# theodorblackbird/lina-speech

Hardware: AMD Instinct MI355X
Metric: codec tokens/sec (whole node), 169M d1024xl12 batched greedy decode (higher is better)
Workload: dtype bf16

## Files before the change

### lina-speech_amd/csrc/gla_decode_window.hip

```cpp
#include <lina_dev.h>
#include "lina_common.h"
#include "skinny_frag.h"

#ifndef LINA_K1W_HIST_NT
#define LINA_K1W_HIST_NT 0
#endif

#ifndef LINA_K1W_STATE_PLAIN
#define LINA_K1W_STATE_PLAIN 0
#endif
#ifndef LINA_K1W_NO_TAIL_LOADS
#define LINA_K1W_NO_TAIL_LOADS 0
#endif
#if LINA_K1W_STATE_PLAIN
#define LINA_K1W_STATE_LOAD(p) (*reinterpret_cast<const float4*>(p))
#else
#define LINA_K1W_STATE_LOAD(p) ld_nt4(p)
#endif

namespace lina {

constexpr int kWinMax = 16;

__device__ __forceinline__ float ld_hist(const float* p) {
#if LINA_K1W_HIST_NT
    return ld_nt1(p);
#else
    return *p;
#endif
}
__device__ __forceinline__ void st_hist(float* p, float v) {
#if LINA_K1W_HIST_NT
    st_nt1(p, v);
#else
    *p = v;
#endif
}

template <typename TS> struct state_piece { static constexpr int n = 4; };
template <> struct state_piece<bf16_t> { static constexpr int n = 8; };
__device__ __forceinline__ void ld_state(const float* p, float (&x)[4]) {
    const float4 t = LINA_K1W_STATE_LOAD(p);
    x[0] = t.x; x[1] = t.y; x[2] = t.z; x[3] = t.w;
}
__device__ __forceinline__ void ld_state(const bf16_t* p, float (&x)[8]) {
    const uint4 u = ld_nt16(p);
    const float4 lo = cvt4(make_uint2(u.x, u.y)), hi = cvt4(make_uint2(u.z, u.w));
    x[0] = lo.x; x[1] = lo.y; x[2] = lo.z; x[3] = lo.w; x[4] = hi.x; x[5] = hi.y; x[6] = hi.z; x[7] = hi.w;
}
__device__ __forceinline__ void st_state(float* p, const float (&x)[4]) { st_nt4(p, make_float4(x[0], x[1], x[2], x[3])); }
__device__ __forceinline__ void st_state(bf16_t* p, const float (&x)[8]) {
    st_nt16(p, make_uint4(pack_bf16x2(x[0], x[1]), pack_bf16x2(x[2], x[3]), pack_bf16x2(x[4], x[5]), pack_bf16x2(x[6], x[7])));
}

template <int DV, int NRB, int CS, typename TIO, typename TG, typename TS = float>
__global__ __launch_bounds__(256 * NRB) void gla_decode_window_kernel(
    const TIO* __restrict__ q, const TIO* __restrict__ k, const TIO* __restrict__ v, const TG* __restrict__ gk, TS* S,
    float* hist_k, float* hist_c, float* hist_v, const int64_t* step, const int64_t* origin, int window, int flush_n,
    int H, int64_t q_sb, int64_t q_sh, int64_t k_sb, int64_t k_sh, int64_t v_sb, int64_t v_sh, int64_t g_sb,
    int64_t g_sh, float scale, const TIO* __restrict__ gate, int64_t gate_sb, int64_t gate_sh,
    const TIO* __restrict__ nw, float eps, TIO* __restrict__ og, int og_packed, float* o_x, int* counters) {
    constexpr int DVT = DV * CS;
    constexpr int RB = 64;
    constexpr int DK = RB * NRB;
    constexpr int EPL = state_piece<TS>::n;
    constexpr int CG = DV / EPL;
    constexpr int RPI = 256 / CG;
    constexpr int NP = RB / RPI;
    __shared__ float s_q[DK], s_e[DK], s_a[kWinMax][NRB];
    __shared__ float s_w[kWinMax][DK];
    __shared__ __attribute__((aligned(16))) float s_v[kWinMax][DV];
    __shared__ __attribute__((aligned(16))) float s_red[NRB * RPI * DV];

    const int tid = threadIdx.x;
    const int rb = tid >> 8, t256 = tid & 255;
    const int cg = t256 % CG, rg = t256 / CG;
    const int bh = blockIdx.x, b = bh / H, h = bh % H;
    const int r0 = rb * RB;
    const int64_t BH = gridDim.x;
    const int col0 = CS > 1 ? (int)blockIdx.y * DV : 0;
    TS* tile = S + ((int64_t)bh * DK + r0) * DVT + col0 + EPL * cg;

    const bool flush_only = flush_n >= 0;
    const int j = flush_only ? flush_n - 1 : ((int)(step[0] - origin[0]) & (window - 1));
    const bool write_back = flush_only || j == window - 1;
    if (flush_only && flush_n == 0) return;

    const int n_hist = flush_only ? j + 1 : j;
    constexpr int NV = 192 * NRB;
    const bool row_wave = t256 < RB;
    float h1[kWinMax], h2[kWinMax];
    float gj = 0.f, kj = 0.f, qj = 0.f, vj = 0.f;
    const int row = r0 + (t256 & (RB - 1));
    const int64_t hoff = (int64_t)bh * DK + row;
    const int vc = rb * 192 + t256 - RB;
    if (row_wave) {
#pragma unroll
        for (int s = 0; s < kWinMax; ++s) {
            h1[s] = s < n_hist ? ld_hist(&hist_c[(int64_t)s * BH * DK + hoff]) : 0.0f;
            h2[s] = s < n_hist ? ld_hist(&hist_k[(int64_t)s * BH * DK + hoff]) : 0.0f;
        }
        if (!flush_only) {
            gj = ld(gk + b * g_sb + h * g_sh + row);
            kj = ld(k + b * k_sb + h * k_sh + row);
            qj = ld(q + b * q_sb + h * q_sh + row) * scale;
        }
    } else if (vc < DV) {
#pragma unroll
        for (int s = 0; s < kWinMax; ++s) h1[s] = s < n_hist ? ld_hist(&hist_v[((int64_t)s * BH + bh) * DVT + col0 + vc]) : 0.0f;
        if (!flush_only) vj = ld(v + b * v_sb + h * v_sh + col0 + vc);
    }

    float St[NP][EPL];
#pragma unroll
    for (int i = 0; i < NP; ++i) ld_state(tile + (int64_t)(rg + RPI * i) * DVT, St[i]);

    if (row_wave) {
        float cj;
        if (flush_only) {
            cj = h1[kWinMax - 1];
#pragma unroll
            for (int s = 0; s < kWinMax - 1; ++s) cj = (s == j) ? h1[s] : cj;
        } else {
            float cprev = 0.0f;
#pragma unroll
            for (int s = 0; s < kWinMax; ++s) cprev = (s == j - 1) ? h1[s] : cprev;
            cj = cprev + gj;
            if (CS == 1 || blockIdx.y == 0) {
                st_hist(&hist_c[(int64_t)j * BH * DK + hoff], cj);
                st_hist(&hist_k[(int64_t)j * BH * DK + hoff], kj);
            }
        }
        s_q[row] = qj;
        s_e[row] = __expf(cj);
#pragma unroll
        for (int s = 0; s < kWinMax; ++s) {
            if (s <= j) {
                const float ws = (!flush_only && s == j) ? kj : __expf(cj - h1[s]) * h2[s];
                s_w[s][row] = ws;
                float a = qj * ws;
                a += shfl_xor(a, 1); a += shfl_xor(a, 2); a += shfl_xor(a, 4);
                a += shfl_xor(a, 8); a += shfl_xor(a, 16); a += shfl_xor(a, 32);
                if (t256 == 0) s_a[s][rb] = a;
            }
        }
    } else {
        if (vc < DV) {
#pragma unroll
            for (int s = 0; s < kWinMax; ++s)
                if (s <= j) s_v[s][vc] = (!flush_only && s == j) ? vj : h1[s];
            if (!flush_only) st_hist(&hist_v[((int64_t)j * BH + bh) * DVT + col0 + vc], vj);
        }
        for (int c = vc + NV; c < DV; c += NV) {
            for (int s = 0; s <= j; ++s) {
                float vs;
                if (!flush_only && s == j) {
                    vs = ld(v + b * v_sb + h * v_sh + col0 + c);
                    hist_v[((int64_t)j * BH + bh) * DVT + col0 + c] = vs;
                } else {
                    vs = hist_v[((int64_t)s * BH + bh) * DVT + col0 + c];
                }
                s_v[s][c] = vs;
            }
        }
    }
    __syncthreads();

    float acc[EPL];
#pragma unroll
    for (int e = 0; e < EPL; ++e) acc[e] = 0.f;
    if (write_back) {
#pragma unroll
        for (int i = 0; i < NP; ++i) {
            const float d = s_e[r0 + rg + RPI * i];
#pragma unroll
            for (int e = 0; e < EPL; ++e) St[i][e] *= d;
        }
        for (int s = 0; s <= j; ++s) {
            float vv[EPL];
#pragma unroll
            for (int e4 = 0; e4 < EPL; e4 += 4) {
                const float4 t = *reinterpret_cast<const float4*>(&s_v[s][EPL * cg + e4]);
                vv[e4] = t.x; vv[e4 + 1] = t.y; vv[e4 + 2] = t.z; vv[e4 + 3] = t.w;
            }
#pragma unroll
            for (int i = 0; i < NP; ++i) {
                const float ws = s_w[s][r0 + rg + RPI * i];
#pragma unroll
                for (int e = 0; e < EPL; ++e) St[i][e] = fmaf(ws, vv[e], St[i][e]);
            }
        }
#pragma unroll
        for (int i = 0; i < NP; ++i) st_state(tile + (int64_t)(rg + RPI * i) * DVT, St[i]);
        if (flush_only) return;
#pragma unroll
        for (int i = 0; i < NP; ++i) {
            const float qq = s_q[r0 + rg + RPI * i];
#pragma unroll
            for (int e = 0; e < EPL; ++e) acc[e] = fmaf(qq, St[i][e], acc[e]);
        }
    } else {
#pragma unroll
        for (int i = 0; i < NP; ++i) {
            const int rr = r0 + rg + RPI * i;
            const float qe = s_q[rr] * s_e[rr];
#pragma unroll
            for (int e = 0; e < EPL; ++e) acc[e] = fmaf(qe, St[i][e], acc[e]);
        }
    }
#pragma unroll
    for (int e4 = 0; e4 < EPL; e4 += 4)
        *reinterpret_cast<float4*>(&s_red[(rb * RPI + rg) * DV + EPL * cg + e4]) = make_float4(acc[e4], acc[e4 + 1], acc[e4 + 2], acc[e4 + 3]);
    __syncthreads();
    if (tid < 64) {
        constexpr int CG4 = DV / 4;
        float4 r = make_float4(0.f, 0.f, 0.f, 0.f);
        if (tid < CG4) {
            r = *reinterpret_cast<const float4*>(&s_red[4 * tid]);
#pragma unroll
            for (int jj = 1; jj < NRB * RPI; ++jj) {
                const float4 t = *reinterpret_cast<const float4*>(&s_red[jj * DV + 4 * tid]);
                r.x += t.x; r.y += t.y; r.z += t.z; r.w += t.w;
            }
            if (!write_back)
                for (int s = 0; s <= j; ++s) {
                    float a = s_a[s][0];
#pragma unroll
                    for (int g2 = 1; g2 < NRB; ++g2) a += s_a[s][g2];
                    const float4 vv = *reinterpret_cast<const float4*>(&s_v[s][4 * tid]);
                    r.x = fmaf(a, vv.x, r.x); r.y = fmaf(a, vv.y, r.y); r.z = fmaf(a, vv.z, r.z); r.w = fmaf(a, vv.w, r.w);
                }
        }
        float ss = r.x * r.x + r.y * r.y + r.z * r.z + r.w * r.w;
        ss += shfl_xor(ss, 1); ss += shfl_xor(ss, 2); ss += shfl_xor(ss, 4);
        ss += shfl_xor(ss, 8); ss += shfl_xor(ss, 16); ss += shfl_xor(ss, 32);
        auto finish = [&](float4 x, int c0, float rs) {
            if (tid < CG4) {
                x.x *= rs; x.y *= rs; x.z *= rs; x.w *= rs;
#if LINA_K1W_NO_TAIL_LOADS
                const float4 ww = make_float4(1.f, 1.f, 1.f, 1.f), gg = make_float4(eps, scale, eps, scale);
#else
                const float4 ww = ld4(nw + c0 + 4 * tid);
                const float4 gg = ld4(gate + b * gate_sb + h * gate_sh + c0 + 4 * tid);
#endif
                x.x *= ww.x; x.y *= ww.y; x.z *= ww.z; x.w *= ww.w;
                x.x *= gg.x * sigmoidf(gg.x); x.y *= gg.y * sigmoidf(gg.y);
                x.z *= gg.z * sigmoidf(gg.z); x.w *= gg.w * sigmoidf(gg.w);
                if (og_packed) st4(og + packed_off<TIO>(b, h * DVT + c0 + 4 * tid, H * DVT), x);
                else st4(og + (int64_t)bh * DVT + c0 + 4 * tid, x);
            }
        };
        if constexpr (CS == 1) {
            finish(r, 0, rsqrtf(ss / (float)DV + eps));
        } else {
            float* ox = o_x + (int64_t)bh * DVT;
            if (tid < CG4) { st_agent8(ox + col0 + 4 * tid, r.x, r.y); st_agent8(ox + col0 + 4 * tid + 2, r.z, r.w); }
            drain_stores();
            int t = 0;
            if (tid == 0) t = ticket_agent(&counters[bh]);
            t = shfl_i(t, 0);
            if (t == CS - 1) {
                if (tid == 0) counters[bh] = 0;
                float4 oth[CS];
                float tot = ss;
#pragma unroll
                for (int c = 0; c < CS; ++c) {
                    oth[c] = r;
                    if (c != (int)blockIdx.y) {
                        float4 x = make_float4(0.f, 0.f, 0.f, 0.f);
                        if (tid < CG4) {
                            const float2 lo = ld_agent8(ox + c * DV + 4 * tid), hi = ld_agent8(ox + c * DV + 4 * tid + 2);
                            x = make_float4(lo.x, lo.y, hi.x, hi.y);
                        }
                        float s2 = x.x * x.x + x.y * x.y + x.z * x.z + x.w * x.w;
                        s2 += shfl_xor(s2, 1); s2 += shfl_xor(s2, 2); s2 += shfl_xor(s2, 4);
                        s2 += shfl_xor(s2, 8); s2 += shfl_xor(s2, 16); s2 += shfl_xor(s2, 32);
                        tot += s2;
                        oth[c] = x;
                    }
                }
                const float rs = rsqrtf(tot / (float)DVT + eps);
#pragma unroll
                for (int c = 0; c < CS; ++c) finish(oth[c], c * DV, rs);
            }
        }
    }
}

constexpr int kWinPersist = 8;
template <typename T> __device__ __forceinline__ T* at_byte(T* base, int byte_off) {
    opaque(byte_off);
    return (T*)((const char*)base + (unsigned)byte_off);
}

template <int DV, int NRB, int CS, typename TIO, typename TG, typename TS = float>
__global__ __launch_bounds__(256 * NRB) void gla_decode_window_persist_kernel(
    const TIO* __restrict__ q, const TIO* __restrict__ k, const TIO* __restrict__ v, const TG* __restrict__ gk, TS* S,
    float* hist_k, float* hist_c, float* hist_v, const int64_t* step, const int64_t* origin, int window, int n_heads,
    int H, int64_t q_sb, int64_t q_sh, int64_t k_sb, int64_t k_sh, int64_t v_sb, int64_t v_sh, int64_t g_sb,
    int64_t g_sh, float scale, const TIO* __restrict__ gate, int64_t gate_sb, int64_t gate_sh,
    const TIO* __restrict__ nw, float eps, TIO* __restrict__ og, int og_packed) {
    static_assert(CS == 1, "the persistent form serves heads of one column block");
    constexpr int RB = 64;
    constexpr int DK = RB * NRB;
    constexpr int EPL = state_piece<TS>::n;
    constexpr int CG = DV / EPL;
    constexpr int RPI = 256 / CG;
    constexpr int NP = RB / RPI;
    constexpr int RD = NP >= 2 ? NP / 2 : 1;
    constexpr int PG = RD < 4 ? RD : 4;
    static_assert(NP % RD == 0 && RD % PG == 0, "a head is a whole number of passes over the ring");
    constexpr int CG4 = DV / 4;
    constexpr int NH = kWinPersist - 1;
    struct __attribute__((aligned(16))) head_lds {
        __attribute__((aligned(16))) float v[kWinPersist][DV];
        __attribute__((aligned(16))) float red[NRB * RPI * DV];
        float w[kWinPersist][DK];
        float q[DK], e[DK], a[kWinPersist][NRB];
        typename raw4<TIO>::type gate[CG4];
    };
    __shared__ head_lds s_buf[2];
    __shared__ typename raw4<TIO>::type s_nw[CG4];

    const int tid = threadIdx.x;
    const int rb = tid >> 8, t256 = tid & 255;
    const int cg = t256 % CG, rg = t256 / CG;
    const int r0 = rb * RB;
    const int64_t BH = n_heads;
    const int n_wg = (int)gridDim.x;
    int bh = blockIdx.x;
    if (bh >= n_heads) return;

    const int j = (int)(step[0] - origin[0]) & (window - 1);
    const bool write_back = j == window - 1;
    const int n_hist = j;
    const int s_last = n_hist > 0 ? n_hist - 1 : 0;
    constexpr int NV = 192 * NRB;
    const bool row_wave = wave_uniform(t256 < RB ? 1 : 0) != 0;
    const int row = r0 + (t256 & (RB - 1));
    const int vc = rb * 192 + t256 - RB;
    const int vcc = vc < 0 ? 0 : (vc < DV ? vc : DV - 1);
    const int toff = ((r0 + rg) * DV + EPL * cg) * (int)sizeof(TS);
    const int hoffl = (row_wave ? row : vcc) * 4;
    const int rowio = row * (int)sizeof(TIO), rowg = row * (int)sizeof(TG), vcio = vcc * (int)sizeof(TIO);
    const int t4io = (tid & (CG4 - 1)) * 4 * (int)sizeof(TIO);
    int pstep_ = RPI * DV;
    opaque(pstep_);
    const int pstep = wave_uniform(pstep_);
    const float* hA = row_wave ? hist_c : hist_v;
    const float* hB = row_wave ? hist_k : hist_v;
    const int64_t hw = row_wave ? DK : DV;

    float h1[NH], h2[NH];
    decltype(ld_raw(gk)) gj_r;
    decltype(ld_raw(q)) kj_r, qj_r, vj_r;
    typename raw4<TIO>::type gate_r;
    if (tid < CG4) s_nw[tid] = ld4_raw(nw + 4 * tid);
    auto small_loads = [&](int hd) __attribute__((always_inline)) {
        const int b = hd / H, h = hd % H;
#pragma unroll
        for (int s = 0; s < NH; ++s) {
            const int sc = s < n_hist ? s : s_last;
            const int64_t o = ((int64_t)sc * BH + hd) * hw;
            h1[s] = ld_hist(at_byte(hA + o, hoffl));
            h2[s] = ld_hist(at_byte(hB + o, hoffl));
        }
        gj_r = ld_raw(at_byte(gk + (b * g_sb + h * g_sh), rowg));
        kj_r = ld_raw(at_byte(k + (b * k_sb + h * k_sh), rowio));
        qj_r = ld_raw(at_byte(q + (b * q_sb + h * q_sh), rowio));
        vj_r = ld_raw(at_byte(v + (b * v_sb + h * v_sh), vcio));
        gate_r = ld4_raw(at_byte(gate + (b * gate_sb + h * gate_sh), t4io));
    };

    float St[RD][EPL];
    small_loads(bh);
    {
        const TS* tile = S + (int64_t)bh * DK * DV;
#pragma unroll
        for (int i = 0; i < RD; ++i) ld_state(at_byte(tile + i * pstep, toff), St[i]);
    }

    auto head = [&](const bool WB, const bool NEXT, const int p, const int nx) __attribute__((always_inline)) {
        const int b = bh / H, h = bh % H;
        const int64_t hoff = (int64_t)bh * DK;
        head_lds& L = s_buf[p];
        if (tid < CG4) L.gate[tid] = gate_r;
        if (row_wave) {
            const float gj = cvt1(gj_r), kj = cvt1(kj_r), qj = cvt1(qj_r) * scale;
            float cprev = 0.0f;
#pragma unroll
            for (int s = 0; s < NH; ++s) cprev = (s == j - 1) ? h1[s] : cprev;
            const float cj = cprev + gj;
            st_hist(at_byte(hist_c + ((int64_t)j * BH * DK + hoff), row * 4), cj);
            st_hist(at_byte(hist_k + ((int64_t)j * BH * DK + hoff), row * 4), kj);
            L.q[row] = qj;
            L.e[row] = __expf(cj);
#pragma unroll
            for (int s = 0; s < kWinPersist; ++s) {
                if (s <= j) {
                    const float ws = (s == j) ? kj : __expf(cj - h1[s < NH ? s : 0]) * h2[s < NH ? s : 0];
                    L.w[s][row] = ws;
                    float a = qj * ws;
                    a += shfl_xor(a, 1); a += shfl_xor(a, 2); a += shfl_xor(a, 4);
                    a += shfl_xor(a, 8); a += shfl_xor(a, 16); a += shfl_xor(a, 32);
                    if (t256 == 0) L.a[s][rb] = a;
                }
            }
        } else {
            if (vc < DV) {
                const float vj = cvt1(vj_r);
#pragma unroll
                for (int s = 0; s < kWinPersist; ++s)
                    if (s <= j) L.v[s][vc] = (s == j) ? vj : h1[s < NH ? s : 0];
                st_hist(at_byte(hist_v + ((int64_t)j * BH + bh) * DV, vc * 4), vj);
            }
            for (int c = vc + NV; c < DV; c += NV) {
                for (int s = 0; s <= j; ++s) {
                    float vs;
                    if (s == j) {
                        vs = ld(v + b * v_sb + h * v_sh + c);
                        hist_v[((int64_t)j * BH + bh) * DV + c] = vs;
                    } else {
                        vs = hist_v[((int64_t)s * BH + bh) * DV + c];
                    }
                    L.v[s][c] = vs;
                }
            }
        }
        __syncthreads();

        small_loads(NEXT ? nx : bh);
        TS* tile = S + (int64_t)bh * DK * DV;
        const TS* tile_nx = NEXT ? S + (int64_t)nx * DK * DV : tile;
        const int pstep_nx = NEXT ? pstep : 0;

        float acc[EPL];
#pragma unroll
        for (int e = 0; e < EPL; ++e) acc[e] = 0.f;
#pragma unroll
        for (int g0 = 0; g0 < NP; g0 += PG) {
            const int sl = g0 % RD;
            if (WB) {
#pragma unroll
                for (int u = 0; u < PG; ++u) {
                    const float d = L.e[r0 + rg + RPI * (g0 + u)];
#pragma unroll
                    for (int e = 0; e < EPL; ++e) St[sl + u][e] *= d;
                }
                for (int s = 0; s <= j; ++s) {
                    float vv[EPL];
#pragma unroll
                    for (int e4 = 0; e4 < EPL; e4 += 4) {
                        const float4 t = *reinterpret_cast<const float4*>(&L.v[s][EPL * cg + e4]);
                        vv[e4] = t.x; vv[e4 + 1] = t.y; vv[e4 + 2] = t.z; vv[e4 + 3] = t.w;
                    }
#pragma unroll
                    for (int u = 0; u < PG; ++u) {
                        const float ws = L.w[s][r0 + rg + RPI * (g0 + u)];
#pragma unroll
                        for (int e = 0; e < EPL; ++e) St[sl + u][e] = fmaf(ws, vv[e], St[sl + u][e]);
                    }
                }
#pragma unroll
                for (int u = 0; u < PG; ++u) st_state(at_byte(tile + (g0 + u) * pstep, toff), St[sl + u]);
#pragma unroll
                for (int u = 0; u < PG; ++u) {
                    const float qq = L.q[r0 + rg + RPI * (g0 + u)];
#pragma unroll
                    for (int e = 0; e < EPL; ++e) acc[e] = fmaf(qq, St[sl + u][e], acc[e]);
                }
            } else {
#pragma unroll
                for (int u = 0; u < PG; ++u) {
                    const int rr = r0 + rg + RPI * (g0 + u);
                    const float qe = L.q[rr] * L.e[rr];
#pragma unroll
                    for (int e = 0; e < EPL; ++e) acc[e] = fmaf(qe, St[sl + u][e], acc[e]);
                }
            }
            if (g0 + RD < NP) {
#pragma unroll
                for (int u = 0; u < PG; ++u) ld_state(at_byte(tile + (g0 + RD + u) * pstep, toff), St[sl + u]);
            } else {
#pragma unroll
                for (int u = 0; u < PG; ++u) ld_state(at_byte(tile_nx + (g0 + RD - NP + u) * pstep_nx, toff), St[sl + u]);
            }
        }
#pragma unroll
        for (int e4 = 0; e4 < EPL; e4 += 4)
            *reinterpret_cast<float4*>(&L.red[(rb * RPI + rg) * DV + EPL * cg + e4]) = make_float4(acc[e4], acc[e4 + 1], acc[e4 + 2], acc[e4 + 3]);
        __syncthreads();
        if (tid < 64) {
            float4 r = make_float4(0.f, 0.f, 0.f, 0.f);
            if (tid < CG4) {
                r = *reinterpret_cast<const float4*>(&L.red[4 * tid]);
#pragma unroll
                for (int jj = 1; jj < NRB * RPI; ++jj) {
                    const float4 t = *reinterpret_cast<const float4*>(&L.red[jj * DV + 4 * tid]);
                    r.x += t.x; r.y += t.y; r.z += t.z; r.w += t.w;
                }
                if (!WB)
                    for (int s = 0; s <= j; ++s) {
                        float a = L.a[s][0];
#pragma unroll
                        for (int g2 = 1; g2 < NRB; ++g2) a += L.a[s][g2];
                        const float4 vv = *reinterpret_cast<const float4*>(&L.v[s][4 * tid]);
                        r.x = fmaf(a, vv.x, r.x); r.y = fmaf(a, vv.y, r.y); r.z = fmaf(a, vv.z, r.z); r.w = fmaf(a, vv.w, r.w);
                    }
            }
            float ss = r.x * r.x + r.y * r.y + r.z * r.z + r.w * r.w;
            ss += shfl_xor(ss, 1); ss += shfl_xor(ss, 2); ss += shfl_xor(ss, 4);
            ss += shfl_xor(ss, 8); ss += shfl_xor(ss, 16); ss += shfl_xor(ss, 32);
            if (tid < CG4) {
                const float rs = rsqrtf(ss / (float)DV + eps);
                float4 x = r;
                x.x *= rs; x.y *= rs; x.z *= rs; x.w *= rs;
                const float4 ww = cvt4(s_nw[tid]), gg = cvt4(L.gate[tid]);
                x.x *= ww.x; x.y *= ww.y; x.z *= ww.z; x.w *= ww.w;
                x.x *= gg.x * sigmoidf(gg.x); x.y *= gg.y * sigmoidf(gg.y);
                x.z *= gg.z * sigmoidf(gg.z); x.w *= gg.w * sigmoidf(gg.w);
                if (og_packed) st4(og + packed_off<TIO>(b, h * DV + 4 * tid, H * DV), x);
                else st4(og + (int64_t)bh * DV + 4 * tid, x);
            }
        }
    };

    for (int p = 0;; p ^= 1) {
        const int nx = bh + n_wg;
        const bool has_next = nx < n_heads;
        head(write_back, has_next, p, nx);
        if (!has_next) break;
        bh = nx;
    }
}

template <typename TIO, typename TG, typename TS = float>
static int launch_window(const void* q, const void* k, const void* v, const void* gk, TS* S, float* hk, float* hc,
                         float* hv, const int64_t* step, const int64_t* origin, int window, int flush_n, int B, int H,
                         int Dk, int Dv, const int64_t* st, float scale, lina_stream_t stream, const void* gate,
                         int64_t gate_sb, int64_t gate_sh, const void* nw, float eps, void* og, int og_packed = 0,
                         float* o_x = nullptr, int* counters = nullptr) {
    const int cs = Dv == 512 ? 2 : 1;
    dim3 grid((unsigned)(B * H), (unsigned)cs);
#define LINA_WIN_ONE(DVV, NRBB, CSS)                                                                                   \
    LINA_LAUNCH((gla_decode_window_kernel<DVV, NRBB, CSS, TIO, TG, TS>), grid, dim3(256 * NRBB), 0, stream, (const TIO*)q, \
                (const TIO*)k, (const TIO*)v, (const TG*)gk, S, hk, hc, hv, step, origin, window, flush_n, H, st[0],   \
                st[1], st[2], st[3], st[4], st[5], st[6], st[7], scale, (const TIO*)gate, gate_sb, gate_sh,            \
                (const TIO*)nw, eps, (TIO*)og, og_packed, o_x, counters)
#define LINA_WIN_CASE(DVV)                                                                                             \
    case DVV:                                                                                                          \
        if (Dk == 64) LINA_WIN_ONE(DVV, 1, 1); else if (Dk == 128) LINA_WIN_ONE(DVV, 2, 1); else LINA_WIN_ONE(DVV, 4, 1); \
        break;
    if (Dk != 64 && Dk != 128 && Dk != 256)
        return fail(LINA_ERR_UNSUPPORTED, "lina_gla_decode_window: Dk=%d not in {64,128,256}", Dk);
    if (cs == 2 && flush_n < 0 && !(o_x && counters))
        return fail(LINA_ERR_ARG, "lina_gla_decode_window: Dv=512 needs the o_exchange buffer and the counters");
    switch (Dv) {
        LINA_WIN_CASE(64) LINA_WIN_CASE(128) LINA_WIN_CASE(256)
        case 512:
            if (Dk == 64) LINA_WIN_ONE(256, 1, 2); else if (Dk == 128) LINA_WIN_ONE(256, 2, 2); else LINA_WIN_ONE(256, 4, 2);
            break;
        default: return fail(LINA_ERR_UNSUPPORTED, "lina_gla_decode_window: Dv=%d not in {64,128,256,512}", Dv);
    }
#undef LINA_WIN_CASE
#undef LINA_WIN_ONE
    return check_launch("lina_gla_decode_window");
}

template <typename TIO, typename TG, typename TS>
static int launch_window_persist(const void* q, const void* k, const void* v, const void* gk, TS* S, float* hk, float* hc,
                                 float* hv, const int64_t* step, const int64_t* origin, int window, int n_wg, int B, int H,
                                 int Dk, int Dv, const int64_t* st, float scale, lina_stream_t stream, const void* gate,
                                 int64_t gate_sb, int64_t gate_sh, const void* nw, float eps, void* og, int og_packed) {
    const int n_heads = B * H;
    dim3 grid((unsigned)(n_wg < n_heads ? n_wg : n_heads));
#define LINA_WINP_ONE(DVV, NRBB)                                                                                       \
    LINA_LAUNCH((gla_decode_window_persist_kernel<DVV, NRBB, 1, TIO, TG, TS>), grid, dim3(256 * NRBB), 0, stream,      \
                (const TIO*)q, (const TIO*)k, (const TIO*)v, (const TG*)gk, S, hk, hc, hv, step, origin, window, n_heads, \
                H, st[0], st[1], st[2], st[3], st[4], st[5], st[6], st[7], scale, (const TIO*)gate, gate_sb, gate_sh,  \
                (const TIO*)nw, eps, (TIO*)og, og_packed)
#define LINA_WINP_CASE(DVV)                                                                                            \
    case DVV:                                                                                                          \
        if (Dk == 64) LINA_WINP_ONE(DVV, 1); else if (Dk == 128) LINA_WINP_ONE(DVV, 2);                                \
        else if constexpr (sizeof(TIO) == 2) LINA_WINP_ONE(DVV, 4);                                                    \
        break;
    if (Dk != 64 && Dk != 128 && Dk != 256)
        return fail(LINA_ERR_UNSUPPORTED, "lina_gla_decode_window_persist: Dk=%d not in {64,128,256}", Dk);
    if (Dk == 256 && sizeof(TIO) != 2)
        return fail(LINA_ERR_UNSUPPORTED, "lina_gla_decode_window_persist: Dk=256 is built for bf16 activations (fp32: "
                    "lina_gla_decode_window_s)");
    switch (Dv) {
        LINA_WINP_CASE(64) LINA_WINP_CASE(128) LINA_WINP_CASE(256)
        default:
            return fail(LINA_ERR_UNSUPPORTED, "lina_gla_decode_window_persist: Dv=%d not in {64,128,256} (Dv = 512 is served by "
                        "lina_gla_decode_window_s)", Dv);
    }
#undef LINA_WINP_CASE
#undef LINA_WINP_ONE
    return check_launch("lina_gla_decode_window_persist");
}

}

extern "C" int lina_gla_decode_window_max(void) { return lina::kWinMax; }

extern "C" int lina_gla_decode_window(const void* q, const void* k, const void* v, const void* gk,
                                      float* state, const void* gate, const void* norm_weight, void* og,
                                      float* o_exchange, int* counters, float* hist_k, float* hist_c, float* hist_v, const int64_t* step,
                                      const int64_t* origin, int window, int B, int H, int Dk, int Dv, int64_t q_sb,
                                      int64_t q_sh, int64_t k_sb, int64_t k_sh, int64_t v_sb, int64_t v_sh, int64_t g_sb,
                                      int64_t g_sh, int64_t gate_sb, int64_t gate_sh, float eps, int og_packed, int dtype,
                                      int g_dtype, float scale, lina_stream_t stream) {
    using namespace lina;
    LINA_REQUIRE(q && k && v && gk && state && gate && norm_weight && og && hist_k && hist_c && hist_v && step && origin,
                 "lina_gla_decode_window: null pointer");
    LINA_REQUIRE(B > 0 && H > 0, "lina_gla_decode_window: B,H must be positive");
    LINA_REQUIRE(window >= 1 && window <= kWinMax && (window & (window - 1)) == 0,
                 "lina_gla_decode_window: window must be a power of two in [1, %d]", kWinMax);
    LINA_REQUIRE(valid_dtype(dtype) && valid_dtype(g_dtype), "lina_gla_decode_window: bad dtype enum");
    LINA_REQUIRE(gate_sb % 4 == 0 && gate_sh % 4 == 0, "lina_gla_decode_window: gate strides must be multiples of 4");
    const int64_t st[8] = {q_sb, q_sh, k_sb, k_sh, v_sb, v_sh, g_sb, g_sh};
    if (dtype == LINA_F32 && g_dtype == LINA_F32)
        return launch_window<float, float>(q, k, v, gk, state, hist_k, hist_c, hist_v, step, origin, window, -1, B, H,
                                           Dk, Dv, st, scale, stream, gate, gate_sb, gate_sh, norm_weight, eps, og, og_packed,
                                           o_exchange, counters);
    if (dtype == LINA_BF16 && g_dtype == LINA_F32)
        return launch_window<bf16_t, float>(q, k, v, gk, state, hist_k, hist_c, hist_v, step, origin, window, -1, B,
                                            H, Dk, Dv, st, scale, stream, gate, gate_sb, gate_sh, norm_weight, eps, og, og_packed,
                                           o_exchange, counters);
    if (dtype == LINA_BF16 && g_dtype == LINA_BF16)
        return launch_window<bf16_t, bf16_t>(q, k, v, gk, state, hist_k, hist_c, hist_v, step, origin, window, -1, B,
                                             H, Dk, Dv, st, scale, stream, gate, gate_sb, gate_sh, norm_weight, eps, og, og_packed,
                                           o_exchange, counters);
    return fail(LINA_ERR_UNSUPPORTED, "lina_gla_decode_window: dtype=f32 with bf16 gates is not built");
}

extern "C" int lina_gla_decode_window_flush(float* state, const float* hist_k, const float* hist_c, const float* hist_v,
                                            int n_pending, int B, int H, int Dk, int Dv, lina_stream_t stream) {
    using namespace lina;
    LINA_REQUIRE(state && hist_k && hist_c && hist_v, "lina_gla_decode_window_flush: null pointer");
    LINA_REQUIRE(B > 0 && H > 0, "lina_gla_decode_window_flush: B,H must be positive");
    LINA_REQUIRE(n_pending >= 0 && n_pending <= kWinMax, "lina_gla_decode_window_flush: n_pending must be in [0, %d]", kWinMax);
    if (n_pending == 0) return LINA_OK;
    const int64_t st[8] = {0, 0, 0, 0, 0, 0, 0, 0};
    return launch_window<float, float>(nullptr, nullptr, nullptr, nullptr, state, (float*)hist_k, (float*)hist_c,
                                       (float*)hist_v, nullptr, nullptr, kWinMax, n_pending, B, H, Dk, Dv, st, 1.0f, stream,
                                       nullptr, 0, 0, nullptr, 0.f, nullptr);
}

extern "C" int lina_gla_decode_window_s(const void* q, const void* k, const void* v, const void* gk, void* state, int state_dtype,
                                        const void* gate, const void* norm_weight, void* og, float* o_exchange, int* counters,
                                        float* hist_k, float* hist_c, float* hist_v, const int64_t* step, const int64_t* origin,
                                        int window, int B, int H, int Dk, int Dv, int64_t q_sb, int64_t q_sh, int64_t k_sb,
                                        int64_t k_sh, int64_t v_sb, int64_t v_sh, int64_t g_sb, int64_t g_sh, int64_t gate_sb,
                                        int64_t gate_sh, float eps, int og_packed, int dtype, int g_dtype, float scale,
                                        lina_stream_t stream) {
    using namespace lina;
    LINA_REQUIRE(valid_dtype(state_dtype), "lina_gla_decode_window_s: bad state dtype %d", state_dtype);
    if (state_dtype == LINA_F32)
        return lina_gla_decode_window(q, k, v, gk, (float*)state, gate, norm_weight, og, o_exchange, counters, hist_k, hist_c, hist_v,
                                      step, origin, window, B, H, Dk, Dv, q_sb, q_sh, k_sb, k_sh, v_sb, v_sh, g_sb, g_sh, gate_sb,
                                      gate_sh, eps, og_packed, dtype, g_dtype, scale, stream);
    LINA_REQUIRE(q && k && v && gk && state && gate && norm_weight && og && hist_k && hist_c && hist_v && step && origin,
                 "lina_gla_decode_window_s: null pointer");
    LINA_REQUIRE(B > 0 && H > 0, "lina_gla_decode_window_s: B,H must be positive");
    LINA_REQUIRE(window >= 1 && window <= kWinMax && (window & (window - 1)) == 0,
                 "lina_gla_decode_window_s: window must be a power of two in [1, %d]", kWinMax);
    LINA_REQUIRE(valid_dtype(dtype) && valid_dtype(g_dtype), "lina_gla_decode_window_s: bad dtype enum");
    LINA_REQUIRE(gate_sb % 4 == 0 && gate_sh % 4 == 0, "lina_gla_decode_window_s: gate strides must be multiples of 4");
    if (dtype != LINA_BF16) return fail(LINA_ERR_UNSUPPORTED, "lina_gla_decode_window_s: a bf16 state is built for bf16 activations");
    const int64_t st[8] = {q_sb, q_sh, k_sb, k_sh, v_sb, v_sh, g_sb, g_sh};
    if (g_dtype == LINA_F32)
        return launch_window<bf16_t, float, bf16_t>(q, k, v, gk, (bf16_t*)state, hist_k, hist_c, hist_v, step, origin, window, -1,
                                                    B, H, Dk, Dv, st, scale, stream, gate, gate_sb, gate_sh, norm_weight, eps, og,
                                                    og_packed, o_exchange, counters);
    return launch_window<bf16_t, bf16_t, bf16_t>(q, k, v, gk, (bf16_t*)state, hist_k, hist_c, hist_v, step, origin, window, -1, B,
                                                 H, Dk, Dv, st, scale, stream, gate, gate_sb, gate_sh, norm_weight, eps, og,
                                                 og_packed, o_exchange, counters);
}

extern "C" int lina_gla_decode_window_flush_s(void* state, int state_dtype, const float* hist_k, const float* hist_c,
                                              const float* hist_v, int n_pending, int B, int H, int Dk, int Dv,
                                              lina_stream_t stream) {
    using namespace lina;
    LINA_REQUIRE(valid_dtype(state_dtype), "lina_gla_decode_window_flush_s: bad state dtype %d", state_dtype);
    if (state_dtype == LINA_F32)
        return lina_gla_decode_window_flush((float*)state, hist_k, hist_c, hist_v, n_pending, B, H, Dk, Dv, stream);
    LINA_REQUIRE(state && hist_k && hist_c && hist_v, "lina_gla_decode_window_flush_s: null pointer");
    LINA_REQUIRE(B > 0 && H > 0, "lina_gla_decode_window_flush_s: B,H must be positive");
    LINA_REQUIRE(n_pending >= 0 && n_pending <= kWinMax, "lina_gla_decode_window_flush_s: n_pending must be in [0, %d]", kWinMax);
    if (n_pending == 0) return LINA_OK;
    const int64_t st[8] = {0, 0, 0, 0, 0, 0, 0, 0};
    return launch_window<bf16_t, float, bf16_t>(nullptr, nullptr, nullptr, nullptr, (bf16_t*)state, (float*)hist_k, (float*)hist_c,
                                                (float*)hist_v, nullptr, nullptr, kWinMax, n_pending, B, H, Dk, Dv, st, 1.0f,
                                                stream, nullptr, 0, 0, nullptr, 0.f, nullptr);
}

extern "C" int lina_gla_decode_window_persist(const void* q, const void* k, const void* v, const void* gk, void* state,
                                              int state_dtype, const void* gate, const void* norm_weight, void* og,
                                              float* o_exchange, int* counters,
                                              float* hist_k, float* hist_c, float* hist_v, const int64_t* step,
                                              const int64_t* origin, int window, int B, int H, int Dk, int Dv, int64_t q_sb,
                                              int64_t q_sh, int64_t k_sb, int64_t k_sh, int64_t v_sb, int64_t v_sh,
                                              int64_t g_sb, int64_t g_sh, int64_t gate_sb, int64_t gate_sh, float eps,
                                              int og_packed, int dtype, int g_dtype, float scale, int n_wg,
                                              lina_stream_t stream) {
    using namespace lina;
    LINA_REQUIRE(valid_dtype(state_dtype), "lina_gla_decode_window_persist: bad state dtype %d", state_dtype);
    LINA_REQUIRE(q && k && v && gk && state && gate && norm_weight && og && hist_k && hist_c && hist_v && step && origin,
                 "lina_gla_decode_window_persist: null pointer");
    LINA_REQUIRE(B > 0 && H > 0, "lina_gla_decode_window_persist: B,H must be positive");
    LINA_REQUIRE(n_wg >= 1, "lina_gla_decode_window_persist: n_wg must be at least 1 (got %d)", n_wg);
    LINA_REQUIRE(window >= 1 && window <= kWinMax && (window & (window - 1)) == 0,
                 "lina_gla_decode_window_persist: window must be a power of two in [1, %d]", kWinMax);
    if (window > kWinPersist)
        return fail(LINA_ERR_UNSUPPORTED, "lina_gla_decode_window_persist: window=%d > %d is served by lina_gla_decode_window_s", window, kWinPersist);
    LINA_REQUIRE(valid_dtype(dtype) && valid_dtype(g_dtype), "lina_gla_decode_window_persist: bad dtype enum");
    LINA_REQUIRE(gate_sb % 4 == 0 && gate_sh % 4 == 0, "lina_gla_decode_window_persist: gate strides must be multiples of 4");
    const int64_t st[8] = {q_sb, q_sh, k_sb, k_sh, v_sb, v_sh, g_sb, g_sh};
#define LINA_WINP_GO(TIO, TG, TS)                                                                                      \
    return launch_window_persist<TIO, TG, TS>(q, k, v, gk, (TS*)state, hist_k, hist_c, hist_v, step, origin, window, n_wg, B, \
                                              H, Dk, Dv, st, scale, stream, gate, gate_sb, gate_sh, norm_weight, eps, og, og_packed)
    if (state_dtype == LINA_F32) {
        if (dtype == LINA_F32 && g_dtype == LINA_F32) LINA_WINP_GO(float, float, float);
        if (dtype == LINA_BF16 && g_dtype == LINA_F32) LINA_WINP_GO(bf16_t, float, float);
        if (dtype == LINA_BF16 && g_dtype == LINA_BF16) LINA_WINP_GO(bf16_t, bf16_t, float);
        return fail(LINA_ERR_UNSUPPORTED, "lina_gla_decode_window_persist: dtype=f32 with bf16 gates is not built");
    }
    if (dtype != LINA_BF16) return fail(LINA_ERR_UNSUPPORTED, "lina_gla_decode_window_persist: a bf16 state is built for bf16 activations");
    if (g_dtype == LINA_F32) LINA_WINP_GO(bf16_t, float, bf16_t);
    LINA_WINP_GO(bf16_t, bf16_t, bf16_t);
#undef LINA_WINP_GO
}
```

Measured before the change: 245,700.

## Stage window history through LDS with wave-wide float4 loads and stores

History reads for c, k and v across the window are redistributed so that each wave issues 16-byte vector loads of whole rows. The results are staged into a new double-buffered LDS region, replacing per-thread scalar loads kept in registers. Writes of the current step's history also become float4 row stores from LDS, done by designated waves after the barrier, and the scalar tail loop over v history is removed. The change trades extra LDS footprint and an added sync for fewer, wider global transactions and lower register pressure, and it now requires the history buffers to be 16-byte aligned.

```diff
diff --git a/lina-speech_amd/csrc/gla_decode_window.hip b/lina-speech_amd/csrc/gla_decode_window.hip
--- a/lina-speech_amd/csrc/gla_decode_window.hip
+++ b/lina-speech_amd/csrc/gla_decode_window.hip
@@ -312,10 +312,14 @@
     static_assert(NP % RD == 0 && RD % PG == 0, "a head is a whole number of passes over the ring");
     constexpr int CG4 = DV / 4;
     constexpr int NH = kWinPersist - 1;
+    constexpr int NW = 4 * NRB;
+    constexpr int NL = (3 * NH + NW - 1) / NW;
     struct __attribute__((aligned(16))) head_lds {
         __attribute__((aligned(16))) float v[kWinPersist][DV];
+        __attribute__((aligned(16))) float ck[2][NH][DK];
         __attribute__((aligned(16))) float red[NRB * RPI * DV];
-        float w[kWinPersist][DK];
+        __attribute__((aligned(16))) float w[kWinPersist][DK];
+        __attribute__((aligned(16))) float c[DK];
         float q[DK], e[DK], a[kWinPersist][NRB];
         typename raw4<TIO>::type gate[CG4];
     };
@@ -337,21 +341,40 @@
     const int s_last = n_hist > 0 ? n_hist - 1 : 0;
     constexpr int NV = 192 * NRB;
     const bool row_wave = wave_uniform(t256 < RB ? 1 : 0) != 0;
+    const int wv = wave_uniform(tid >> 6), lane = tid & 63;
     const int row = r0 + (t256 & (RB - 1));
     const int vc = rb * 192 + t256 - RB;
     const int vcc = vc < 0 ? 0 : (vc < DV ? vc : DV - 1);
     const int toff = ((r0 + rg) * DV + EPL * cg) * (int)sizeof(TS);
-    const int hoffl = (row_wave ? row : vcc) * 4;
+    const int hoffk = (4 * lane < DK ? lane : 0) * 16, hoffv = (4 * lane < DV ? lane : 0) * 16;
     const int rowio = row * (int)sizeof(TIO), rowg = row * (int)sizeof(TG), vcio = vcc * (int)sizeof(TIO);
     const int t4io = (tid & (CG4 - 1)) * 4 * (int)sizeof(TIO);
     int pstep_ = RPI * DV;
     opaque(pstep_);
     const int pstep = wave_uniform(pstep_);
-    const float* hA = row_wave ? hist_c : hist_v;
-    const float* hB = row_wave ? hist_k : hist_v;
-    const int64_t hw = row_wave ? DK : DV;
-
-    float h1[NH], h2[NH];
+
+    const float* hsrc[NL];
+    int hwid[NL], hdst[NL];
+    bool hok[NL];
+#pragma unroll
+    for (int t = 0; t < NL; ++t) {
+        const int pc = wv + NW * t, s = pc / 3, kind = pc - 3 * s;
+        const int sc = s < n_hist ? s : s_last;
+        hwid[t] = kind == 2 ? DV : DK;
+        hsrc[t] = (kind == 0 ? hist_c : (kind == 1 ? hist_k : hist_v)) + (int64_t)sc * BH * hwid[t];
+        hok[t] = s < n_hist;
+        const int sd = s < NH ? s : 0;
+        hdst[t] = kind == 2 ? (int)(__builtin_offsetof(head_lds, v) / 4) + sd * DV
+                            : (int)(__builtin_offsetof(head_lds, ck) / 4) + (kind * NH + sd) * DK;
+    }
+    const int st_kind = wv - (NW - 3);
+    const int st_wid = st_kind == 2 ? DV : DK;
+    float* const st_base = (st_kind <= 0 ? hist_c : (st_kind == 1 ? hist_k : hist_v)) + (int64_t)j * BH * st_wid;
+    const int st_src = st_kind <= 0 ? (int)(__builtin_offsetof(head_lds, c) / 4)
+                                    : (st_kind == 1 ? (int)(__builtin_offsetof(head_lds, w) / 4) + j * DK
+                                                    : (int)(__builtin_offsetof(head_lds, v) / 4) + j * DV);
+
+    float4 hraw[NL];
     decltype(ld_raw(gk)) gj_r;
     decltype(ld_raw(q)) kj_r, qj_r, vj_r;
     typename raw4<TIO>::type gate_r;
@@ -359,18 +382,20 @@
     auto small_loads = [&](int hd) __attribute__((always_inline)) {
         const int b = hd / H, h = hd % H;
 #pragma unroll
-        for (int s = 0; s < NH; ++s) {
-            const int sc = s < n_hist ? s : s_last;
-            const int64_t o = ((int64_t)sc * BH + hd) * hw;
-            h1[s] = ld_hist(at_byte(hA + o, hoffl));
-            h2[s] = ld_hist(at_byte(hB + o, hoffl));
-        }
+        for (int t = 0; t < NL; ++t)
+            hraw[t] = ld4_raw(at_byte(hsrc[t] + (int64_t)hd * hwid[t], hwid[t] == DK ? hoffk : hoffv));
         gj_r = ld_raw(at_byte(gk + (b * g_sb + h * g_sh), rowg));
         kj_r = ld_raw(at_byte(k + (b * k_sb + h * k_sh), rowio));
         qj_r = ld_raw(at_byte(q + (b * q_sb + h * q_sh), rowio));
         vj_r = ld_raw(at_byte(v + (b * v_sb + h * v_sh), vcio));
         gate_r = ld4_raw(at_byte(gate + (b * gate_sb + h * gate_sh), t4io));
     };
+    auto stage = [&](int pb) __attribute__((always_inline)) {
+        float* Lf = reinterpret_cast<float*>(&s_buf[pb]);
+#pragma unroll
+        for (int t = 0; t < NL; ++t)
+            if (hok[t] && 4 * lane < hwid[t]) *reinterpret_cast<float4*>(Lf + hdst[t] + 4 * lane) = hraw[t];
+    };
 
     float St[RD][EPL];
     small_loads(bh);
@@ -379,26 +404,26 @@
 #pragma unroll
         for (int i = 0; i < RD; ++i) ld_state(at_byte(tile + i * pstep, toff), St[i]);
     }
+    stage(0);
+    __syncthreads();
 
     auto head = [&](const bool WB, const bool NEXT, const int p, const int nx) __attribute__((always_inline)) {
         const int b = bh / H, h = bh % H;
-        const int64_t hoff = (int64_t)bh * DK;
         head_lds& L = s_buf[p];
         if (tid < CG4) L.gate[tid] = gate_r;
         if (row_wave) {
             const float gj = cvt1(gj_r), kj = cvt1(kj_r), qj = cvt1(qj_r) * scale;
             float cprev = 0.0f;
-#pragma unroll
-            for (int s = 0; s < NH; ++s) cprev = (s == j - 1) ? h1[s] : cprev;
+            if (j > 0) cprev = L.ck[0][j - 1][row];
             const float cj = cprev + gj;
-            st_hist(at_byte(hist_c + ((int64_t)j * BH * DK + hoff), row * 4), cj);
-            st_hist(at_byte(hist_k + ((int64_t)j * BH * DK + hoff), row * 4), kj);
+            L.c[row] = cj;
             L.q[row] = qj;
             L.e[row] = __expf(cj);
 #pragma unroll
             for (int s = 0; s < kWinPersist; ++s) {
                 if (s <= j) {
-                    const float ws = (s == j) ? kj : __expf(cj - h1[s < NH ? s : 0]) * h2[s < NH ? s : 0];
+                    float ws = kj;
+                    if (s < j) ws = __expf(cj - L.ck[0][s < NH ? s : 0][row]) * L.ck[1][s < NH ? s : 0][row];
                     L.w[s][row] = ws;
                     float a = qj * ws;
                     a += shfl_xor(a, 1); a += shfl_xor(a, 2); a += shfl_xor(a, 4);
@@ -407,27 +432,15 @@
                 }
             }
         } else {
-            if (vc < DV) {
-                const float vj = cvt1(vj_r);
-#pragma unroll
-                for (int s = 0; s < kWinPersist; ++s)
-                    if (s <= j) L.v[s][vc] = (s == j) ? vj : h1[s < NH ? s : 0];
-                st_hist(at_byte(hist_v + ((int64_t)j * BH + bh) * DV, vc * 4), vj);
-            }
-            for (int c = vc + NV; c < DV; c += NV) {
-                for (int s = 0; s <= j; ++s) {
-                    float vs;
-                    if (s == j) {
-                        vs = ld(v + b * v_sb + h * v_sh + c);
-                        hist_v[((int64_t)j * BH + bh) * DV + c] = vs;
-                    } else {
-                        vs = hist_v[((int64_t)s * BH + bh) * DV + c];
-                    }
-                    L.v[s][c] = vs;
-                }
-            }
+            if (vc < DV) L.v[j][vc] = cvt1(vj_r);
+            for (int c = vc + NV; c < DV; c += NV)
+                L.v[j][c] = ld(v + b * v_sb + h * v_sh + c);
         }
         __syncthreads();
+
+        if (st_kind >= 0 && 4 * lane < st_wid)
+            *reinterpret_cast<float4*>(at_byte(st_base + (int64_t)bh * st_wid, lane * 16)) =
+                *reinterpret_cast<const float4*>(reinterpret_cast<const float*>(&L) + st_src + 4 * lane);
 
         small_loads(NEXT ? nx : bh);
         TS* tile = S + (int64_t)bh * DK * DV;
@@ -489,6 +502,7 @@
 #pragma unroll
         for (int e4 = 0; e4 < EPL; e4 += 4)
             *reinterpret_cast<float4*>(&L.red[(rb * RPI + rg) * DV + EPL * cg + e4]) = make_float4(acc[e4], acc[e4 + 1], acc[e4 + 2], acc[e4 + 3]);
+        stage(p ^ 1);
         __syncthreads();
         if (tid < 64) {
             float4 r = make_float4(0.f, 0.f, 0.f, 0.f);
@@ -716,6 +730,8 @@
     if (window > kWinPersist)
         return fail(LINA_ERR_UNSUPPORTED, "lina_gla_decode_window_persist: window=%d > %d is served by lina_gla_decode_window_s", window, kWinPersist);
     LINA_REQUIRE(valid_dtype(dtype) && valid_dtype(g_dtype), "lina_gla_decode_window_persist: bad dtype enum");
+    LINA_REQUIRE((((uintptr_t)hist_k | (uintptr_t)hist_c | (uintptr_t)hist_v) & 15) == 0,
+                 "lina_gla_decode_window_persist: hist_k / hist_c / hist_v must be 16-byte aligned");
     LINA_REQUIRE(gate_sb % 4 == 0 && gate_sh % 4 == 0, "lina_gla_decode_window_persist: gate strides must be multiples of 4");
     const int64_t st[8] = {q_sb, q_sh, k_sb, k_sh, v_sb, v_sh, g_sb, g_sh};
 #define LINA_WINP_GO(TIO, TG, TS)                                                                                      \
```

New measurement: 244,800. About the same (-0.4%).
